# sunnyHelen/JPerceiver

Hardware: AMD Instinct MI355X
Metric: train images/sec (full train step, synthetic 3-frame batches) (higher is better)
Workload: dtype f32

## Files before the change

### jperceiver_amd/csrc/pointwise.hip

```cpp
#include "jp_common.h"
#include "bilinear.h"
#include <algorithm>

namespace {

constexpr int TPB = 256;
inline int blocks_for(long n) { return (int)std::min<long>((n + TPB - 1) / TPB, 1 << 20); }

constexpr int MP_TW = 64, MP_TH = 8;

__global__ __launch_bounds__(TPB) void maxpool_fwd_kernel(const float* __restrict__ x, float* __restrict__ y,
                                                          uint8_t* __restrict__ idx, int H, int W, int OH, int OW,
                                                          int k, int s, int p) {
    extern __shared__ float tile[];
    const size_t nc = blockIdx.z;
    const float* xp = x + nc * H * W;
    const int ox0 = blockIdx.x * MP_TW, oy0 = blockIdx.y * MP_TH;
    const int pw = (MP_TW - 1) * s + k, ph = (MP_TH - 1) * s + k;
    const int ix0 = ox0 * s - p, iy0 = oy0 * s - p;
    for (int i = threadIdx.x; i < pw * ph; i += TPB) {
        const int ly = i / pw, lx = i - ly * pw;
        const int iy = iy0 + ly, ix = ix0 + lx;
        tile[i] = ((unsigned)iy < (unsigned)H && (unsigned)ix < (unsigned)W) ? xp[iy * W + ix] : -INFINITY;
    }
    __syncthreads();
    for (int o = threadIdx.x; o < MP_TW * MP_TH; o += TPB) {
        const int ty = o / MP_TW, tx = o - ty * MP_TW;
        const int oy = oy0 + ty, ox = ox0 + tx;
        if (oy >= OH || ox >= OW) continue;
        float best = -INFINITY;
        int bi = -1;
        for (int ky = 0; ky < k; ++ky) {
            const float* row = tile + (ty * s + ky) * pw + tx * s;
            const bool rin = (unsigned)(iy0 + ty * s + ky) < (unsigned)H;
            for (int kx = 0; kx < k; ++kx) {
                const float v = row[kx];
                const bool in = rin && (unsigned)(ix0 + tx * s + kx) < (unsigned)W;
                if (in && (bi < 0 || v > best || v != v)) { best = v; bi = ky * k + kx; }
            }
        }
        y[nc * OH * OW + oy * OW + ox] = best;
        idx[nc * OH * OW + oy * OW + ox] = (uint8_t)max(bi, 0);
    }
}

__global__ __launch_bounds__(TPB) void maxpool_bwd_kernel(const float* __restrict__ dy,
                                                          const uint8_t* __restrict__ idx, float* __restrict__ dx,
                                                          const float* __restrict__ addend, int H, int W, int OH,
                                                          int OW, int k, int s, int p, int pw, int ph) {
    extern __shared__ float tile[];
    int* itile = reinterpret_cast<int*>(tile + pw * ph);
    const size_t nc = blockIdx.z;
    const float* dp = dy + nc * OH * OW;
    const uint8_t* ip = idx + nc * OH * OW;
    const int ix0 = blockIdx.x * MP_TW, iy0 = blockIdx.y * MP_TH;
    int oy0 = iy0 + p - k + 1;
    oy0 = oy0 <= 0 ? 0 : (oy0 + s - 1) / s;
    int ox0 = ix0 + p - k + 1;
    ox0 = ox0 <= 0 ? 0 : (ox0 + s - 1) / s;
    for (int i = threadIdx.x; i < pw * ph; i += TPB) {
        const int ly = i / pw, lx = i - ly * pw;
        const int oy = oy0 + ly, ox = ox0 + lx;
        const bool in = oy < OH && ox < OW;
        tile[i] = in ? dp[oy * OW + ox] : 0.f;
        itile[i] = in ? (int)ip[oy * OW + ox] : -1;
    }
    __syncthreads();
    for (int o = threadIdx.x; o < MP_TW * MP_TH; o += TPB) {
        const int ty = o / MP_TW, tx = o - ty * MP_TW;
        const int iy = iy0 + ty, ix = ix0 + tx;
        if (iy >= H || ix >= W) continue;
        int oy_lo = iy + p - k + 1;
        oy_lo = oy_lo <= 0 ? 0 : (oy_lo + s - 1) / s;
        const int oy_hi = min(OH - 1, (iy + p) / s);
        int ox_lo = ix + p - k + 1;
        ox_lo = ox_lo <= 0 ? 0 : (ox_lo + s - 1) / s;
        const int ox_hi = min(OW - 1, (ix + p) / s);
        float g = 0.f;
        for (int oy = oy_lo; oy <= oy_hi; ++oy) {
            const int ky = iy - (oy * s - p);
            for (int ox = ox_lo; ox <= ox_hi; ++ox) {
                const int kx = ix - (ox * s - p);
                const int li = (oy - oy0) * pw + (ox - ox0);
                if (itile[li] == ky * k + kx) g += tile[li];
            }
        }
        if (addend) g += addend[nc * H * W + iy * W + ix];
        dx[nc * H * W + iy * W + ix] = g;
    }
}

constexpr int MPF_TH = 16;
template <int K, int S>
__global__ __launch_bounds__(TPB) void maxpool_fwd_t_kernel(const float* __restrict__ x, float* __restrict__ y,
                                                            uint8_t* __restrict__ idx, int H, int W, int OH, int OW,
                                                            int p) {
    constexpr int PW = (MP_TW - 1) * S + K, PH = (MPF_TH - 1) * S + K;
    __shared__ float tile[PW * PH];
    const size_t nc = blockIdx.z;
    const float* xp = x + nc * H * W;
    const int ox0 = blockIdx.x * MP_TW, oy0 = blockIdx.y * MPF_TH;
    const int ix0 = ox0 * S - p, iy0 = oy0 * S - p;
    for (int i = threadIdx.x; i < PW * PH; i += TPB) {
        const int ly = i / PW, lx = i - ly * PW;
        const int iy = iy0 + ly, ix = ix0 + lx;
        tile[i] = ((unsigned)iy < (unsigned)H && (unsigned)ix < (unsigned)W) ? xp[iy * W + ix] : -INFINITY;
    }
    __syncthreads();
    const int tx = threadIdx.x & 63, q = threadIdx.x >> 6;
    float best[4];
    int bi[4];
#pragma unroll
    for (int j = 0; j < 4; ++j) { best[j] = -INFINITY; bi[j] = 0; }
    const float* base = tile + (q * 4 * S) * PW + tx * S;
    constexpr int R = 3 * S + K;
#pragma unroll
    for (int r = 0; r < R; ++r) {
        float rv = base[r * PW];
        int rk = 0;
#pragma unroll
        for (int kx = 1; kx < K; ++kx) {
            const float v = base[r * PW + kx];
            const bool take = v > rv || v != v;
            rv = take ? v : rv;
            rk = take ? kx : rk;
        }
#pragma unroll
        for (int j = 0; j < 4; ++j) {
            const int ky = r - j * S;
            if (ky < 0 || ky >= K) continue;
            const bool take = ky == 0 || rv > best[j] || rv != rv;
            best[j] = take ? rv : best[j];
            bi[j] = take ? ky * K + rk : bi[j];
        }
    }
    const int ox = ox0 + tx;
    if (ox >= OW) return;
#pragma unroll
    for (int j = 0; j < 4; ++j) {
        const int oy = oy0 + q * 4 + j;
        if (oy < OH) {
            y[nc * OH * OW + oy * OW + ox] = best[j];
            idx[nc * OH * OW + oy * OW + ox] = (uint8_t)bi[j];
        }
    }
}

template <int K>
__global__ __launch_bounds__(TPB) void maxpool_bwd_s1_kernel(const float* __restrict__ dy,
                                                             const uint8_t* __restrict__ idx, float* __restrict__ dx,
                                                             const float* __restrict__ addend, int H, int W, int OH,
                                                             int OW, int p) {
    constexpr int PW = MP_TW + K - 1, PH = MPF_TH + K - 1;
    __shared__ float tile[PW * PH];
    __shared__ int itile[PW * PH];
    const size_t nc = blockIdx.z;
    const float* dp = dy + nc * OH * OW;
    const uint8_t* ip = idx + nc * OH * OW;
    const int ix0 = blockIdx.x * MP_TW, iy0 = blockIdx.y * MPF_TH;
    const int oy0 = iy0 + p - (K - 1), ox0 = ix0 + p - (K - 1);
    for (int i = threadIdx.x; i < PW * PH; i += TPB) {
        const int ly = i / PW, lx = i - ly * PW;
        const int oy = oy0 + ly, ox = ox0 + lx;
        const bool in = (unsigned)oy < (unsigned)OH && (unsigned)ox < (unsigned)OW;
        tile[i] = in ? dp[oy * OW + ox] : 0.f;
        itile[i] = in ? (int)ip[oy * OW + ox] : -1;
    }
    __syncthreads();
    const int tx = threadIdx.x & 63, q = threadIdx.x >> 6;
    const int ix = ix0 + tx;
    if (ix >= W) return;
#pragma unroll
    for (int j = 0; j < 4; ++j) {
        const int ty = q * 4 + j, iy = iy0 + ty;
        if (iy >= H) break;
        float g = 0.f;
#pragma unroll
        for (int ky = 0; ky < K; ++ky)
#pragma unroll
            for (int kx = 0; kx < K; ++kx) {
                const int li = (ty + K - 1 - ky) * PW + tx + K - 1 - kx;
                g += itile[li] == ky * K + kx ? tile[li] : 0.f;
            }
        if (addend) g += addend[nc * H * W + iy * W + ix];
        dx[nc * H * W + iy * W + ix] = g;
    }
}

template <int L>
__device__ __forceinline__ void row5_neighbours(const float4 v, int lane_in_row, float e[8], float pad) {
    const float lz = __shfl_up(v.z, 1, 64), lw = __shfl_up(v.w, 1, 64);
    const float rx = __shfl_down(v.x, 1, 64), ry = __shfl_down(v.y, 1, 64);
    e[0] = lane_in_row == 0 ? pad : lz;
    e[1] = lane_in_row == 0 ? pad : lw;
    e[2] = v.x; e[3] = v.y; e[4] = v.z; e[5] = v.w;
    e[6] = lane_in_row == L - 1 ? pad : rx;
    e[7] = lane_in_row == L - 1 ? pad : ry;
}

template <int L>
__global__ __launch_bounds__(TPB) void maxpool5_rows_fwd_kernel(const float* __restrict__ x, float* __restrict__ y,
                                                                uint8_t* __restrict__ idx, int NC, int H, int RB, int bands) {
    constexpr int G = 64 / L, W = 4 * L;
    const int lane = threadIdx.x & 63, wave = threadIdx.x >> 6;
    const int grp = lane / L, lir = lane % L;
    const long unit = ((long)blockIdx.x * 4 + wave) * G + grp;
    const bool live = unit < (long)NC * bands;
    const long nc = live ? unit / bands : 0;
    const int r0 = live ? (int)(unit % bands) * RB : 0;
    const int r1 = min(H, r0 + RB);
    const float4* xp = reinterpret_cast<const float4*>(x + nc * (long)H * W) + lir;
    float4* yp = reinterpret_cast<float4*>(y + nc * (long)H * W) + lir;
    uchar4* ip = reinterpret_cast<uchar4*>(idx + nc * (long)H * W) + lir;
    const float NEG = -INFINITY;
    float rv[5][4];
    int rk[5][4];
#pragma unroll
    for (int i = 0; i < 5; ++i)
#pragma unroll
        for (int j = 0; j < 4; ++j) { rv[i][j] = NEG; rk[i][j] = 0; }
    const int rend = live ? r1 + 2 : r0 - 2;
    for (int r = r0 - 2; r < rend; ++r) {
        float4 v = make_float4(NEG, NEG, NEG, NEG);
        if ((unsigned)r < (unsigned)H) v = xp[(long)r * L];
        float e[8];
        row5_neighbours<L>(v, lir, e, NEG);
#pragma unroll
        for (int i = 0; i < 4; ++i)
#pragma unroll
            for (int j = 0; j < 4; ++j) { rv[i][j] = rv[i + 1][j]; rk[i][j] = rk[i + 1][j]; }
#pragma unroll
        for (int j = 0; j < 4; ++j) {
            float b = e[j];
            int k = 0;
#pragma unroll
            for (int kx = 1; kx < 5; ++kx) {
                const float c = e[j + kx];
                const bool take = c > b || c != c;
                b = take ? c : b;
                k = take ? kx : k;
            }
            rv[4][j] = b;
            rk[4][j] = k;
        }
        const int oy = r - 2;
        if (oy >= r0) {
            float o[4];
            unsigned char oi[4];
#pragma unroll
            for (int j = 0; j < 4; ++j) {
                float b = rv[0][j];
                int bi = rk[0][j];
#pragma unroll
                for (int ky = 1; ky < 5; ++ky) {
                    const float c = rv[ky][j];
                    const bool take = c > b || c != c;
                    b = take ? c : b;
                    bi = take ? ky * 5 + rk[ky][j] : bi;
                }
                o[j] = b;
                oi[j] = (unsigned char)bi;
            }
            yp[(long)oy * L] = make_float4(o[0], o[1], o[2], o[3]);
            ip[(long)oy * L] = make_uchar4(oi[0], oi[1], oi[2], oi[3]);
        }
    }
}

template <int L>
__global__ __launch_bounds__(TPB) void maxpool5_rows_bwd_kernel(const float* __restrict__ dy, const uint8_t* __restrict__ idx,
                                                                float* __restrict__ dx, const float* __restrict__ addend,
                                                                int NC, int H, int RB, int bands, unsigned* __restrict__ amax) {
    constexpr int G = 64 / L, W = 4 * L;
    float mx = 0.f;
    const int lane = threadIdx.x & 63, wave = threadIdx.x >> 6;
    const int grp = lane / L, lir = lane % L;
    const long unit = ((long)blockIdx.x * 4 + wave) * G + grp;
    const bool live = unit < (long)NC * bands;
    const long nc = live ? unit / bands : 0;
    const int r0 = live ? (int)(unit % bands) * RB : 0;
    const int r1 = min(H, r0 + RB);
    const float4* dp = reinterpret_cast<const float4*>(dy + nc * (long)H * W) + lir;
    const uchar4* ip = reinterpret_cast<const uchar4*>(idx + nc * (long)H * W) + lir;
    const float4* ap = addend ? reinterpret_cast<const float4*>(addend + nc * (long)H * W) + lir : nullptr;
    float4* op = reinterpret_cast<float4*>(dx + nc * (long)H * W) + lir;
    float d[5][4];
    int wy[5][4], wx[5][4];
#pragma unroll
    for (int i = 0; i < 5; ++i)
#pragma unroll
        for (int j = 0; j < 4; ++j) { d[i][j] = 0.f; wy[i][j] = 7; wx[i][j] = 0; }
    const int oend = live ? r1 + 2 : r0 - 2;
    for (int oy = r0 - 2; oy < oend; ++oy) {
#pragma unroll
        for (int i = 0; i < 4; ++i)
#pragma unroll
            for (int j = 0; j < 4; ++j) { d[i][j] = d[i + 1][j]; wy[i][j] = wy[i + 1][j]; wx[i][j] = wx[i + 1][j]; }
        if ((unsigned)oy < (unsigned)H) {
            const float4 g = dp[(long)oy * L];
            const uchar4 q = ip[(long)oy * L];
            const float gg[4] = {g.x, g.y, g.z, g.w};
            const int qq[4] = {q.x, q.y, q.z, q.w};
#pragma unroll
            for (int j = 0; j < 4; ++j) {
                const int ky = (qq[j] * 13) >> 6;
                d[4][j] = gg[j];
                wy[4][j] = ky;
                wx[4][j] = qq[j] - 5 * ky;
            }
        } else {
#pragma unroll
            for (int j = 0; j < 4; ++j) { d[4][j] = 0.f; wy[4][j] = 7; wx[4][j] = 0; }
        }
        const int r = oy - 2;
        float t[4];
        float tk[4];
#pragma unroll
        for (int j = 0; j < 4; ++j) {
            float acc = 0.f;
            int kx = 0;
#pragma unroll
            for (int i = 0; i < 5; ++i) {
                const bool hit = wy[i][j] == 4 - i;
                acc += hit ? d[i][j] : 0.f;
                kx = hit ? wx[i][j] : kx;
            }
            t[j] = acc;
            tk[j] = (float)kx;
        }
        float et[8], ek[8];
        row5_neighbours<L>(make_float4(t[0], t[1], t[2], t[3]), lir, et, 0.f);
        row5_neighbours<L>(make_float4(tk[0], tk[1], tk[2], tk[3]), lir, ek, -1.f);
        if (r >= r0 && r < r1) {
            float o[4];
#pragma unroll
            for (int j = 0; j < 4; ++j) {
                float acc = 0.f;
#pragma unroll
                for (int m = 0; m < 5; ++m) acc += ek[j + m] == (float)(4 - m) ? et[j + m] : 0.f;
                o[j] = acc;
            }
            if (ap) { const float4 a = ap[(long)r * L]; o[0] += a.x; o[1] += a.y; o[2] += a.z; o[3] += a.w; }
            op[(long)r * L] = make_float4(o[0], o[1], o[2], o[3]);
            mx = fmaxf(fmaxf(mx, fmaxf(jp_fmag(o[0]), jp_fmag(o[1]))), fmaxf(jp_fmag(o[2]), jp_fmag(o[3])));
        }
    }
    jp_wave_amax_commit(mx, amax);
}

__global__ __launch_bounds__(TPB) void maxpool3s2_bwd_kernel(const float* __restrict__ dy, const uint8_t* __restrict__ idx,
                                                             float* __restrict__ dx, const float* __restrict__ addend, long units,
                                                             int OH, int OW, int RB, int bands) {
    const long u = (long)blockIdx.x * TPB + threadIdx.x;
    if (u >= units) return;
    const int OW2 = OW >> 1, W = 2 * OW;
    const int q = (int)(u % OW2);
    const long v = u / OW2;
    const int b = (int)(v % bands);
    const long nc = v / bands;
    const int i0 = b * RB, i1 = min(OH, i0 + RB);
    const float* dp = dy + nc * (long)OH * OW + 2 * q;
    const uint8_t* ip = idx + nc * (long)OH * OW + 2 * q;
    float* op = dx + nc * 4L * OH * OW + 4 * q;
    const float* ap = addend ? addend + nc * 4L * OH * OW + 4 * q : nullptr;
    const bool right = 2 * q + 2 < OW;
    float g[2][3];
    int k[2][3];
    auto load = [&](int slot, int i) {
        if (i < OH) {
            const float2 a = *reinterpret_cast<const float2*>(dp + (long)i * OW);
            const uchar2 c = *reinterpret_cast<const uchar2*>(ip + (long)i * OW);
            g[slot][0] = a.x; g[slot][1] = a.y; k[slot][0] = c.x; k[slot][1] = c.y;
            g[slot][2] = right ? dp[(long)i * OW + 2] : 0.f;
            k[slot][2] = right ? (int)ip[(long)i * OW + 2] : -1;
        } else {
#pragma unroll
            for (int c = 0; c < 3; ++c) { g[slot][c] = 0.f; k[slot][c] = -1; }
        }
    };
    load(0, i0);
    for (int i = i0; i < i1; ++i) {
        load(1, i + 1);
        float4 r0, r1;
        r0.x = k[0][0] == 4 ? g[0][0] : 0.f;
        r0.y = (k[0][0] == 5 ? g[0][0] : 0.f) + (k[0][1] == 3 ? g[0][1] : 0.f);
        r0.z = k[0][1] == 4 ? g[0][1] : 0.f;
        r0.w = (k[0][1] == 5 ? g[0][1] : 0.f) + (k[0][2] == 3 ? g[0][2] : 0.f);
        r1.x = (k[0][0] == 7 ? g[0][0] : 0.f) + (k[1][0] == 1 ? g[1][0] : 0.f);
        r1.y = (k[0][0] == 8 ? g[0][0] : 0.f) + (k[0][1] == 6 ? g[0][1] : 0.f) + (k[1][0] == 2 ? g[1][0] : 0.f) + (k[1][1] == 0 ? g[1][1] : 0.f);
        r1.z = (k[0][1] == 7 ? g[0][1] : 0.f) + (k[1][1] == 1 ? g[1][1] : 0.f);
        r1.w = (k[0][1] == 8 ? g[0][1] : 0.f) + (k[0][2] == 6 ? g[0][2] : 0.f) + (k[1][1] == 2 ? g[1][1] : 0.f) + (k[1][2] == 0 ? g[1][2] : 0.f);
        if (ap) {
            const float4 a0 = *reinterpret_cast<const float4*>(ap + (long)(2 * i) * W);
            const float4 a1 = *reinterpret_cast<const float4*>(ap + (long)(2 * i + 1) * W);
            r0.x += a0.x; r0.y += a0.y; r0.z += a0.z; r0.w += a0.w;
            r1.x += a1.x; r1.y += a1.y; r1.z += a1.z; r1.w += a1.w;
        }
        *reinterpret_cast<float4*>(op + (long)(2 * i) * W) = r0;
        *reinterpret_cast<float4*>(op + (long)(2 * i + 1) * W) = r1;
#pragma unroll
        for (int c = 0; c < 3; ++c) { g[0][c] = g[1][c]; k[0][c] = k[1][c]; }
    }
}

template <int L>
static void launch_pool5_rows(bool fwd, const float* a, float* out, uint8_t* idx, const uint8_t* cidx, const float* addend,
                              int NC, int H, hipStream_t st, unsigned* amax) {
    const int G = 64 / L;
    int RB = H <= 64 ? H : 64;
    while (RB > 16 && (long)NC * jp_cdiv(H, RB) / G < 4096) RB >>= 1;
    const int bands = jp_cdiv(H, RB);
    const long units = (long)NC * bands;
    const dim3 grid((unsigned)jp_cdiv(units, 4L * G));
    if (fwd) hipLaunchKernelGGL((maxpool5_rows_fwd_kernel<L>), grid, dim3(TPB), 0, st, a, out, idx, NC, H, RB, bands);
    else hipLaunchKernelGGL((maxpool5_rows_bwd_kernel<L>), grid, dim3(TPB), 0, st, a, cidx, out, addend, NC, H, RB, bands, amax);
}
static bool pool5_rows_ok(int k, int s, int p, int W) {
    return k == 5 && s == 1 && p == 2 && (W == 32 || W == 64 || W == 128 || W == 256);
}
static void pool5_rows(bool fwd, const float* a, float* out, uint8_t* idx, const uint8_t* cidx, const float* addend, int NC,
                       int H, int W, hipStream_t st, unsigned* amax = nullptr) {
    switch (W) {
        case 32: launch_pool5_rows<8>(fwd, a, out, idx, cidx, addend, NC, H, st, amax); break;
        case 64: launch_pool5_rows<16>(fwd, a, out, idx, cidx, addend, NC, H, st, amax); break;
        case 128: launch_pool5_rows<32>(fwd, a, out, idx, cidx, addend, NC, H, st, amax); break;
        default: launch_pool5_rows<64>(fwd, a, out, idx, cidx, addend, NC, H, st, amax); break;
    }
}

__global__ __launch_bounds__(TPB) void upsample2x_fwd_kernel(const float* __restrict__ x, float* __restrict__ y,
                                                             long total, int C, int H, int W, int dstC, int dc0) {
    const int OW = 2 * W, OH = 2 * H;
    for (long o = (long)blockIdx.x * TPB + threadIdx.x; o < total; o += (long)gridDim.x * TPB) {
        const int ox = (int)(o % OW);
        const long t = o / OW;
        const int oy = (int)(t % OH);
        const long nc = t / OH;
        const int c = (int)(nc % C);
        const long n = nc / C;
        y[((n * dstC + dc0 + c) * OH + oy) * OW + ox] = x[(nc * H + (oy >> 1)) * W + (ox >> 1)];
    }
}

__global__ __launch_bounds__(TPB) void upsample2x_fwd_v4_kernel(const float* __restrict__ x, float* __restrict__ y,
                                                                unsigned total4, int C, int H, int W4, int dstC,
                                                                int dc0) {
    for (unsigned i = blockIdx.x * TPB + threadIdx.x; i < total4; i += gridDim.x * TPB) {
        const unsigned xq = i % W4, t = i / W4;
        const unsigned yy = t % H, nc = t / H;
        const unsigned c = nc % C, n = nc / C;
        const float4 v = reinterpret_cast<const float4*>(x)[i];
        float4* o = reinterpret_cast<float4*>(y + (((size_t)n * dstC + dc0 + c) * (2 * H) + 2 * yy) * (8 * W4)) + 2 * xq;
        const float4 a = make_float4(v.x, v.x, v.y, v.y), b = make_float4(v.z, v.z, v.w, v.w);
        o[0] = a; o[1] = b;
        o[2 * W4] = a; o[2 * W4 + 1] = b;
    }
}

__global__ __launch_bounds__(TPB) void upsample2x_bwd_v2_kernel(const float* __restrict__ dy, float* __restrict__ dx,
                                                                unsigned total2, int C, int H, int W2, int Ctot, int c0,
                                                                int accumulate) {
    for (unsigned i = blockIdx.x * TPB + threadIdx.x; i < total2; i += gridDim.x * TPB) {
        const unsigned xp = i % W2, t = i / W2;
        const unsigned yy = t % H, nc = t / H;
        const unsigned c = nc % C, n = nc / C;
        const float4* d = reinterpret_cast<const float4*>(dy + (((size_t)n * Ctot + c0 + c) * (2 * H) + 2 * yy) * (4 * W2)) + xp;
        const float4 r0 = d[0], r1 = d[W2];
        float2 g = make_float2(r0.x + r0.y + r1.x + r1.y, r0.z + r0.w + r1.z + r1.w);
        float2* o = reinterpret_cast<float2*>(dx) + i;
        if (accumulate) { const float2 p = *o; g.x += p.x; g.y += p.y; }
        *o = g;
    }
}

__global__ __launch_bounds__(TPB) void upsample2x_bwd_kernel(const float* __restrict__ dy, float* __restrict__ dx,
                                                             long total, int C, int H, int W, int Ctot, int c0,
                                                             int accumulate) {
    const int OW = 2 * W;
    for (long i = (long)blockIdx.x * TPB + threadIdx.x; i < total; i += (long)gridDim.x * TPB) {
        const int x = (int)(i % W);
        const long t = i / W;
        const int y = (int)(t % H);
        const long nc = t / H;
        const int c = (int)(nc % C);
        const long n = nc / C;
        const float* d = dy + ((n * Ctot + c0 + c) * (2L * H) + 2 * y) * OW + 2 * x;
        const float g = d[0] + d[1] + d[OW] + d[OW + 1];
        dx[i] = accumulate ? dx[i] + g : g;
    }
}

__global__ __launch_bounds__(TPB) void copy_channels_kernel(const float* __restrict__ src, float* __restrict__ dst,
                                                            long total, int C, int HW, int srcC, int sc0, int dstC,
                                                            int dc0, int accumulate) {
    for (long i = (long)blockIdx.x * TPB + threadIdx.x; i < total; i += (long)gridDim.x * TPB) {
        const int p = (int)(i % HW);
        const long t = i / HW;
        const int c = (int)(t % C);
        const long n = t / C;
        const float v = src[(n * srcC + sc0 + c) * HW + p];
        float* q = dst + (n * dstC + dc0 + c) * HW + p;
        *q = accumulate ? *q + v : v;
    }
}

__global__ __launch_bounds__(TPB) void copy_channels_v4_kernel(const float* __restrict__ src, float* __restrict__ dst,
                                                               unsigned total4, int C, int HW4, int srcC, int sc0,
                                                               int dstC, int dc0, int accumulate) {
    for (unsigned i = blockIdx.x * TPB + threadIdx.x; i < total4; i += gridDim.x * TPB) {
        const unsigned p = i % HW4, t = i / HW4;
        const unsigned c = t % C, n = t / C;
        float4 v = reinterpret_cast<const float4*>(src)[((size_t)n * srcC + sc0 + c) * HW4 + p];
        float4* q = reinterpret_cast<float4*>(dst) + ((size_t)n * dstC + dc0 + c) * HW4 + p;
        if (accumulate) { const float4 o = *q; v.x += o.x; v.y += o.y; v.z += o.z; v.w += o.w; }
        *q = v;
    }
}

template <class F4, class F1>
__device__ __forceinline__ void ew_loop(long n, bool aligned, F4 f4, F1 f1) {
    const long n4 = aligned ? (n >> 2) : 0;
    for (long i = (long)blockIdx.x * TPB + threadIdx.x; i < n4; i += (long)gridDim.x * TPB) f4(i);
    for (long i = (n4 << 2) + (long)blockIdx.x * TPB + threadIdx.x; i < n; i += (long)gridDim.x * TPB) f1(i);
}
__device__ __forceinline__ bool al16(const void* a, const void* b = nullptr, const void* c = nullptr, const void* d = nullptr,
                                     const void* e = nullptr, const void* f = nullptr) {
    return (((uintptr_t)a | (uintptr_t)b | (uintptr_t)c | (uintptr_t)d | (uintptr_t)e | (uintptr_t)f) & 15) == 0;
}
#define JP_F4(p) reinterpret_cast<const float4*>(p)
#define JP_F4W(p) reinterpret_cast<float4*>(p)

__global__ __launch_bounds__(TPB) void axpby_kernel(const float* __restrict__ a, const float* __restrict__ b,
                                                    float* __restrict__ out, long n, float alpha, float beta) {
    ew_loop(n, al16(a, b, out),
            [&](long i) {
                const float4 x = JP_F4(a)[i];
                float4 r = make_float4(alpha * x.x, alpha * x.y, alpha * x.z, alpha * x.w);
                if (b) { const float4 y = JP_F4(b)[i]; r.x += beta * y.x; r.y += beta * y.y; r.z += beta * y.z; r.w += beta * y.w; }
                JP_F4W(out)[i] = r;
            },
            [&](long i) { out[i] = alpha * a[i] + (b ? beta * b[i] : 0.f); });
}

__global__ __launch_bounds__(TPB) void sum_n_kernel(const float* __restrict__ a0, const float* __restrict__ a1,
                                                    const float* __restrict__ a2, const float* __restrict__ a3,
                                                    const float* __restrict__ a4, float* __restrict__ out, long n,
                                                    unsigned* __restrict__ amax) {
    float mx = 0.f;
    ew_loop(n, al16(a0, a1, a2, a3, a4, out),
            [&](long i) {
                float4 r = JP_F4(a0)[i];
                const float4 b = JP_F4(a1)[i];
                r.x += b.x; r.y += b.y; r.z += b.z; r.w += b.w;
                if (a2) { const float4 c = JP_F4(a2)[i]; r.x += c.x; r.y += c.y; r.z += c.z; r.w += c.w; }
                if (a3) { const float4 c = JP_F4(a3)[i]; r.x += c.x; r.y += c.y; r.z += c.z; r.w += c.w; }
                if (a4) { const float4 c = JP_F4(a4)[i]; r.x += c.x; r.y += c.y; r.z += c.z; r.w += c.w; }
                JP_F4W(out)[i] = r;
                mx = fmaxf(fmaxf(mx, fmaxf(jp_fmag(r.x), jp_fmag(r.y))), fmaxf(jp_fmag(r.z), jp_fmag(r.w)));
            },
            [&](long i) {
                float r = a0[i] + a1[i];
                if (a2) r += a2[i];
                if (a3) r += a3[i];
                if (a4) r += a4[i];
                out[i] = r;
                mx = fmaxf(mx, jp_fmag(r));
            });
    jp_block_amax_commit(mx, amax);
}

__global__ __launch_bounds__(TPB) void mul_kernel(const float* __restrict__ a, const float* __restrict__ b,
                                                  float* __restrict__ out, long n, float scale) {
    ew_loop(n, al16(a, b, out),
            [&](long i) {
                const float4 x = JP_F4(a)[i], y = JP_F4(b)[i];
                JP_F4W(out)[i] = make_float4(x.x * y.x * scale, x.y * y.y * scale, x.z * y.z * scale, x.w * y.w * scale);
            },
            [&](long i) { out[i] = a[i] * b[i] * scale; });
}

__global__ __launch_bounds__(TPB) void affine_kernel(const float* __restrict__ a, float* __restrict__ out, long n,
                                                     float scale, float shift) {
    ew_loop(n, al16(a, out),
            [&](long i) {
                const float4 x = JP_F4(a)[i];
                JP_F4W(out)[i] = make_float4(x.x * scale + shift, x.y * scale + shift, x.z * scale + shift, x.w * scale + shift);
            },
            [&](long i) { out[i] = a[i] * scale + shift; });
}

__global__ __launch_bounds__(TPB) void act_fwd_kernel(const float* __restrict__ x, float* __restrict__ y, long n,
                                                      int act) {
    ew_loop(n, al16(x, y),
            [&](long i) {
                const float4 v = JP_F4(x)[i];
                JP_F4W(y)[i] = make_float4(jp_act(v.x, act), jp_act(v.y, act), jp_act(v.z, act), jp_act(v.w, act));
            },
            [&](long i) { y[i] = jp_act(x[i], act); });
}

__device__ __forceinline__ float act_bwd1(float d, float v, int act) {
    if (act == JP_ACT_RELU) return v > 0.f ? d : 0.f;
    if (act == JP_ACT_LEAKY) return v > 0.f ? d : 0.01f * d;
    if (act == JP_ACT_SIGMOID) return d * v * (1.f - v);
    return d;
}
__global__ __launch_bounds__(TPB) void act_bwd_kernel(const float* __restrict__ dy, const float* __restrict__ y,
                                                      float* __restrict__ dx, long n, int act, unsigned* __restrict__ amax) {
    float mx = 0.f;
    ew_loop(n, al16(dy, y, dx),
            [&](long i) {
                const float4 d = JP_F4(dy)[i], v = JP_F4(y)[i];
                const float4 o = make_float4(act_bwd1(d.x, v.x, act), act_bwd1(d.y, v.y, act), act_bwd1(d.z, v.z, act),
                                             act_bwd1(d.w, v.w, act));
                JP_F4W(dx)[i] = o;
                mx = fmaxf(fmaxf(mx, fmaxf(jp_fmag(o.x), jp_fmag(o.y))), fmaxf(jp_fmag(o.z), jp_fmag(o.w)));
            },
            [&](long i) {
                const float o = act_bwd1(dy[i], y[i], act);
                dx[i] = o;
                mx = fmaxf(mx, jp_fmag(o));
            });
    jp_block_amax_commit(mx, amax);
}

__global__ __launch_bounds__(TPB) void act_bwd_bias_kernel(const float* __restrict__ dy, const float* __restrict__ y, float* __restrict__ dx,
                                                           float* __restrict__ dbias, int C, int HW, int CH, int chunk, int act,
                                                           unsigned* __restrict__ amax, float* __restrict__ part) {
    __shared__ double sm[4];
    const int c = blockIdx.x;
    const int n = blockIdx.y / CH, ck = blockIdx.y - n * CH;
    const int beg = ck * chunk, end = min(HW, beg + chunk);
    const size_t base = ((size_t)n * C + c) * HW;
    double s = 0.0;
    float fs = 0.f, mx = 0.f;
    int run = 0;
    if (((HW | chunk) & 3) == 0) {
        const float4* d4 = reinterpret_cast<const float4*>(dy + base);
        const float4* y4 = reinterpret_cast<const float4*>(y + base);
        float4* o4 = reinterpret_cast<float4*>(dx + base);
        for (int i = (beg >> 2) + threadIdx.x; i < (end >> 2); i += TPB) {
            const float4 d = d4[i], v = y4[i];
            const float4 o = make_float4(act_bwd1(d.x, v.x, act), act_bwd1(d.y, v.y, act), act_bwd1(d.z, v.z, act), act_bwd1(d.w, v.w, act));
            o4[i] = o;
            mx = fmaxf(fmaxf(mx, fmaxf(jp_fmag(o.x), jp_fmag(o.y))), fmaxf(jp_fmag(o.z), jp_fmag(o.w)));
            fs += (o.x + o.y) + (o.z + o.w);
            if (++run == 8) { s += fs; fs = 0.f; run = 0; }
        }
    } else {
        for (int i = beg + threadIdx.x; i < end; i += TPB) {
            const float o = act_bwd1(dy[base + i], y[base + i], act);
            dx[base + i] = o;
            mx = fmaxf(mx, jp_fmag(o));
            fs += o;
            if (++run == 32) { s += fs; fs = 0.f; run = 0; }
        }
    }
    jp_block_amax_commit(mx, amax);
    s += fs;
    s = jp_block_sum_d(s, sm);
    if (threadIdx.x == 0) {
        if (part) part[(size_t)c * gridDim.y + blockIdx.y] = (float)s;
        else atomicAdd(&dbias[c], (float)s);
    }
}
__global__ void bias_fold_kernel(const float* __restrict__ part, float* __restrict__ dbias, int C, int S) {
    const int c = blockIdx.x * blockDim.x + threadIdx.x;
    if (c >= C) return;
    float s = 0.f;
    for (int i = 0; i < S; ++i) s += part[(size_t)c * S + i];
    dbias[c] += s;
}

__global__ __launch_bounds__(TPB) void mul_bcast_c_kernel(const float* __restrict__ a, const float* __restrict__ s,
                                                          float* __restrict__ out, long total, int C, int HW) {
    for (long i = (long)blockIdx.x * TPB + threadIdx.x; i < total; i += (long)gridDim.x * TPB) {
        const int p = (int)(i % HW);
        const long n = i / ((long)C * HW);
        out[i] = a[i] * s[n * HW + p];
    }
}
__global__ __launch_bounds__(TPB) void mul_bcast_c_bwd_s_kernel(const float* __restrict__ dout,
                                                                const float* __restrict__ a, float* __restrict__ ds,
                                                                long total, int C, int HW) {
    for (long i = (long)blockIdx.x * TPB + threadIdx.x; i < total; i += (long)gridDim.x * TPB) {
        const int p = (int)(i % HW);
        const long n = i / HW;
        float g = 0.f;
        for (int c = 0; c < C; ++c) g += dout[(n * C + c) * HW + p] * a[(n * C + c) * HW + p];
        ds[i] = g;
    }
}

__global__ __launch_bounds__(TPB) void bilinear_fwd_kernel(const float* __restrict__ x, float* __restrict__ y,
                                                           long total, int H, int W, int OH, int OW, float sy,
                                                           float sx) {
    for (long o = (long)blockIdx.x * TPB + threadIdx.x; o < total; o += (long)gridDim.x * TPB) {
        const int ox = (int)(o % OW);
        const long t = o / OW;
        const int oy = (int)(t % OH);
        const long nc = t / OH;
        y[o] = bil_sample(x + nc * H * W, oy, ox, H, W, sy, sx);
    }
}

__global__ __launch_bounds__(TPB) void bilinear_bwd_kernel(const float* __restrict__ dy, float* __restrict__ dx,
                                                           long total, int H, int W, int OH, int OW, float sy,
                                                           float sx, int accumulate) {
    for (long i = (long)blockIdx.x * TPB + threadIdx.x; i < total; i += (long)gridDim.x * TPB) {
        const int ix = (int)(i % W);
        const long t = i / W;
        const int iy = (int)(t % H);
        const long nc = t / H;
        const float* dp = dy + nc * OH * OW;
        int oy_lo = max(0, (int)floorf(((float)iy - 0.5f) / sy - 0.5f) - 1);
        int oy_hi = min(OH - 1, (int)ceilf(((float)iy + 1.5f) / sy - 0.5f) + 1);
        int ox_lo = max(0, (int)floorf(((float)ix - 0.5f) / sx - 0.5f) - 1);
        int ox_hi = min(OW - 1, (int)ceilf(((float)ix + 1.5f) / sx - 0.5f) + 1);
// ... 497 lines not shown
```

Before: 127.4.

## Software-pipeline row loads in 5x5 maxpool forward and backward kernels

```diff
diff --git a/jperceiver_amd/csrc/pointwise.hip b/jperceiver_amd/csrc/pointwise.hip
--- a/jperceiver_amd/csrc/pointwise.hip
+++ b/jperceiver_amd/csrc/pointwise.hip
@@ -198,10 +198,13 @@
     e[7] = lane_in_row == L - 1 ? pad : ry;
 }
 
-template <int L>
+#define POOL5_LOADS_LANDED() __builtin_amdgcn_s_waitcnt(0x0F70)
+enum { POOL5_FILL = 0, POOL5_STORE = 1, POOL5_TEST = 2 };
+
+template <int L, int AHEAD>
 __global__ __launch_bounds__(TPB) void maxpool5_rows_fwd_kernel(const float* __restrict__ x, float* __restrict__ y,
                                                                 uint8_t* __restrict__ idx, int NC, int H, int RB, int bands) {
-    constexpr int G = 64 / L, W = 4 * L;
+    constexpr int G = 64 / L, W = 4 * L, NB = AHEAD > 0 ? AHEAD : 1;
     const int lane = threadIdx.x & 63, wave = threadIdx.x >> 6;
     const int grp = lane / L, lir = lane % L;
     const long unit = ((long)blockIdx.x * 4 + wave) * G + grp;
@@ -220,9 +223,11 @@
 #pragma unroll
         for (int j = 0; j < 4; ++j) { rv[i][j] = NEG; rk[i][j] = 0; }
     const int rend = live ? r1 + 2 : r0 - 2;
-    for (int r = r0 - 2; r < rend; ++r) {
-        float4 v = make_float4(NEG, NEG, NEG, NEG);
-        if ((unsigned)r < (unsigned)H) v = xp[(long)r * L];
+    const int rlo = max(r0 - 2, 0), rhi = min(r1 + 1, H - 1);
+    auto fetch = [&](int r) { return xp[(long)min(max(r, rlo), rhi) * L]; };
+    auto step = [&](int r, const float4 raw, const int mode) {
+        const bool in = (unsigned)r < (unsigned)H;
+        const float4 v = make_float4(in ? raw.x : NEG, in ? raw.y : NEG, in ? raw.z : NEG, in ? raw.w : NEG);
         float e[8];
         row5_neighbours<L>(v, lir, e, NEG);
 #pragma unroll
@@ -244,7 +249,7 @@
             rk[4][j] = k;
         }
         const int oy = r - 2;
-        if (oy >= r0) {
+        if (mode == POOL5_STORE || (mode == POOL5_TEST && oy >= r0)) {
             float o[4];
             unsigned char oi[4];
 #pragma unroll
@@ -264,14 +269,45 @@
             yp[(long)oy * L] = make_float4(o[0], o[1], o[2], o[3]);
             ip[(long)oy * L] = make_uchar4(oi[0], oi[1], oi[2], oi[3]);
         }
-    }
-}
-
-template <int L>
+    };
+    if constexpr (AHEAD == 0) {
+        for (int r = r0 - 2; r < rend; ++r) {
+            float4 v = make_float4(NEG, NEG, NEG, NEG);
+            if ((unsigned)r < (unsigned)H) v = xp[(long)r * L];
+            step(r, v, POOL5_TEST);
+        }
+    } else if (live) {
+        float4 fill[4], cur[NB], nxt[NB];
+#pragma unroll
+        for (int i = 0; i < 4; ++i) fill[i] = fetch(r0 - 2 + i);
+#pragma unroll
+        for (int i = 0; i < NB; ++i) cur[i] = fetch(r0 + 2 + i);
+#pragma unroll
+        for (int i = 0; i < 4; ++i) step(r0 - 2 + i, fill[i], POOL5_FILL);
+        POOL5_LOADS_LANDED();
+        int rb = r0 + 2;
+#pragma unroll 1
+        for (; rb + NB <= rend; rb += NB) {
+#pragma unroll
+            for (int i = 0; i < NB; ++i) nxt[i] = fetch(rb + NB + i);
+#pragma unroll
+            for (int i = 0; i < NB; ++i) step(rb + i, cur[i], POOL5_STORE);
+#pragma unroll
+            for (int i = 0; i < NB; ++i) cur[i] = nxt[i];
+        }
+#pragma unroll
+        for (int i = 0; i < NB - 1; ++i)
+            if (rb + i < rend) step(rb + i, cur[i], POOL5_STORE);
+    }
+}
+
+struct Pool5BwdRow { float4 g; uchar4 q; float4 a; };
+
+template <int L, int AHEAD, bool ADD>
 __global__ __launch_bounds__(TPB) void maxpool5_rows_bwd_kernel(const float* __restrict__ dy, const uint8_t* __restrict__ idx,
                                                                 float* __restrict__ dx, const float* __restrict__ addend,
                                                                 int NC, int H, int RB, int bands, unsigned* __restrict__ amax) {
-    constexpr int G = 64 / L, W = 4 * L;
+    constexpr int G = 64 / L, W = 4 * L, NB = AHEAD > 0 ? AHEAD : 1;
     float mx = 0.f;
     const int lane = threadIdx.x & 63, wave = threadIdx.x >> 6;
     const int grp = lane / L, lir = lane % L;
@@ -291,16 +327,22 @@
 #pragma unroll
         for (int j = 0; j < 4; ++j) { d[i][j] = 0.f; wy[i][j] = 7; wx[i][j] = 0; }
     const int oend = live ? r1 + 2 : r0 - 2;
-    for (int oy = r0 - 2; oy < oend; ++oy) {
+    const int olo = max(r0 - 2, 0), ohi = min(r1 + 1, H - 1);
+    const float4 zero4 = make_float4(0.f, 0.f, 0.f, 0.f);
+    auto fetch = [&](int oy, bool with_addend) {
+        const long o = (long)min(max(oy, olo), ohi) * L;
+        Pool5BwdRow w = {dp[o], ip[o], zero4};
+        if (ADD && with_addend) w.a = ap[(long)min(max(oy - 2, r0), r1 - 1) * L];
+        return w;
+    };
+    auto step = [&](int oy, const Pool5BwdRow& w, const int mode) {
 #pragma unroll
         for (int i = 0; i < 4; ++i)
 #pragma unroll
             for (int j = 0; j < 4; ++j) { d[i][j] = d[i + 1][j]; wy[i][j] = wy[i + 1][j]; wx[i][j] = wx[i + 1][j]; }
         if ((unsigned)oy < (unsigned)H) {
-            const float4 g = dp[(long)oy * L];
-            const uchar4 q = ip[(long)oy * L];
-            const float gg[4] = {g.x, g.y, g.z, g.w};
-            const int qq[4] = {q.x, q.y, q.z, q.w};
+            const float gg[4] = {w.g.x, w.g.y, w.g.z, w.g.w};
+            const int qq[4] = {w.q.x, w.q.y, w.q.z, w.q.w};
 #pragma unroll
             for (int j = 0; j < 4; ++j) {
                 const int ky = (qq[j] * 13) >> 6;
@@ -331,7 +373,7 @@
         float et[8], ek[8];
         row5_neighbours<L>(make_float4(t[0], t[1], t[2], t[3]), lir, et, 0.f);
         row5_neighbours<L>(make_float4(tk[0], tk[1], tk[2], tk[3]), lir, ek, -1.f);
-        if (r >= r0 && r < r1) {
+        if (mode == POOL5_STORE || (mode == POOL5_TEST && r >= r0 && r < r1)) {
             float o[4];
 #pragma unroll
             for (int j = 0; j < 4; ++j) {
@@ -340,10 +382,42 @@
                 for (int m = 0; m < 5; ++m) acc += ek[j + m] == (float)(4 - m) ? et[j + m] : 0.f;
                 o[j] = acc;
             }
-            if (ap) { const float4 a = ap[(long)r * L]; o[0] += a.x; o[1] += a.y; o[2] += a.z; o[3] += a.w; }
+            if (AHEAD > 0 ? ADD : ap != nullptr) {
+                const float4 a = AHEAD > 0 ? w.a : ap[(long)r * L];
+                o[0] += a.x; o[1] += a.y; o[2] += a.z; o[3] += a.w;
+            }
             op[(long)r * L] = make_float4(o[0], o[1], o[2], o[3]);
             mx = fmaxf(fmaxf(mx, fmaxf(jp_fmag(o[0]), jp_fmag(o[1]))), fmaxf(jp_fmag(o[2]), jp_fmag(o[3])));
         }
+    };
+    if constexpr (AHEAD == 0) {
+        for (int oy = r0 - 2; oy < oend; ++oy) {
+            Pool5BwdRow w = {zero4, make_uchar4(0, 0, 0, 0), zero4};
+            if ((unsigned)oy < (unsigned)H) { w.g = dp[(long)oy * L]; w.q = ip[(long)oy * L]; }
+            step(oy, w, POOL5_TEST);
+        }
+    } else if (live) {
+        Pool5BwdRow fill[4], cur[NB], nxt[NB];
+#pragma unroll
+        for (int i = 0; i < 4; ++i) fill[i] = fetch(r0 - 2 + i, false);
+#pragma unroll
+        for (int i = 0; i < NB; ++i) cur[i] = fetch(r0 + 2 + i, true);
+#pragma unroll
+        for (int i = 0; i < 4; ++i) step(r0 - 2 + i, fill[i], POOL5_FILL);
+        POOL5_LOADS_LANDED();
+        int ob = r0 + 2;
+#pragma unroll 1
+        for (; ob + NB <= oend; ob += NB) {
+#pragma unroll
+            for (int i = 0; i < NB; ++i) nxt[i] = fetch(ob + NB + i, true);
+#pragma unroll
+            for (int i = 0; i < NB; ++i) step(ob + i, cur[i], POOL5_STORE);
+#pragma unroll
+            for (int i = 0; i < NB; ++i) cur[i] = nxt[i];
+        }
+#pragma unroll
+        for (int i = 0; i < NB - 1; ++i)
+            if (ob + i < oend) step(ob + i, cur[i], POOL5_STORE);
     }
     jp_wave_amax_commit(mx, amax);
 }
@@ -403,17 +477,32 @@
     }
 }
 
+constexpr int POOL5_AHEAD_FWD = 3, POOL5_AHEAD_BWD = 2;
+static bool pool5_pipelined() {
+    static const bool on = [] { const char* e = getenv("JP_POOL5_AHEAD"); return !(e && e[0] == '0'); }();
+    return on;
+}
 template <int L>
 static void launch_pool5_rows(bool fwd, const float* a, float* out, uint8_t* idx, const uint8_t* cidx, const float* addend,
                               int NC, int H, hipStream_t st, unsigned* amax) {
+    const bool pipe = pool5_pipelined();
     const int G = 64 / L;
     int RB = H <= 64 ? H : 64;
     while (RB > 16 && (long)NC * jp_cdiv(H, RB) / G < 4096) RB >>= 1;
     const int bands = jp_cdiv(H, RB);
     const long units = (long)NC * bands;
-    const dim3 grid((unsigned)jp_cdiv(units, 4L * G));
-    if (fwd) hipLaunchKernelGGL((maxpool5_rows_fwd_kernel<L>), grid, dim3(TPB), 0, st, a, out, idx, NC, H, RB, bands);
-    else hipLaunchKernelGGL((maxpool5_rows_bwd_kernel<L>), grid, dim3(TPB), 0, st, a, cidx, out, addend, NC, H, RB, bands, amax);
+    const dim3 grid((unsigned)jp_cdiv(units, 4L * G)), block(TPB);
+    constexpr int AF = POOL5_AHEAD_FWD, AB = POOL5_AHEAD_BWD;
+    if (fwd) {
+        if (pipe) hipLaunchKernelGGL((maxpool5_rows_fwd_kernel<L, AF>), grid, block, 0, st, a, out, idx, NC, H, RB, bands);
+        else hipLaunchKernelGGL((maxpool5_rows_fwd_kernel<L, 0>), grid, block, 0, st, a, out, idx, NC, H, RB, bands);
+    } else if (!pipe) {
+        hipLaunchKernelGGL((maxpool5_rows_bwd_kernel<L, 0, false>), grid, block, 0, st, a, cidx, out, addend, NC, H, RB, bands, amax);
+    } else if (addend) {
+        hipLaunchKernelGGL((maxpool5_rows_bwd_kernel<L, AB, true>), grid, block, 0, st, a, cidx, out, addend, NC, H, RB, bands, amax);
+    } else {
+        hipLaunchKernelGGL((maxpool5_rows_bwd_kernel<L, AB, false>), grid, block, 0, st, a, cidx, out, addend, NC, H, RB, bands, amax);
+    }
 }
 static bool pool5_rows_ok(int k, int s, int p, int W) {
     return k == 5 && s == 1 && p == 2 && (W == 32 || W == 64 || W == 128 || W == 256);
```

After: 127.1. Within noise of the previous version (-0.2%).
